# muzishen/RCDMs

Hardware: AMD Instinct MI355X
Metric: story-frames/sec (stage-2 UNet, 50-step DDIM, 512^2) (higher is better)
Workload: dtype f16; 1 GPU; PororoSV stage-2, 512x512, 50-step DDIM, CFG 2.0, batch=1 story x 5 frames per GPU, ctx 85x768, random-init 1276.9M-param UNet3D; stories_per_gpu=1, latent=64, ddim_steps=50, parallelism=story-replicas x1

## Files before the change

rcdms_amd/csrc/rowff.hip:

```cpp
#include "common.h"
#include "pp_sync.h"
#include <type_traits>

#ifndef RCDM_FF_ABLATE
#define RCDM_FF_ABLATE 0
#endif

namespace {

enum { TAIL_FF = 0, TAIL_N1 = 1, TAIL_FFP = 2, TAIL_N3 = 3 };

struct RowArgs {
  const f16* a_in;
  const f16* res;
  f16* tok;
  f16* out;
  const f16* wstream;
  const float* a_bias;
  const float* ln_g;
  const float* ln_b;
  const float* pe;
  const float* b1p;
  const float* b2;
  const f16* z_res;
  const float* z_bias;
  const float* gn_stat;
  const float* gn_g;
  const float* gn_b;
  int M, lda, ldr, ldt, ldo, ldz;
  int rows_per_frame, frames;
  int gn_G, gn_rows;
  float eps;
};

template <int C, int NW, int R, int PD, bool HAS_A, bool A_RES, bool LN_PE, int TAIL>
__global__ __launch_bounds__(NW * 64) void row_chain_kernel(const RowArgs p) {
  constexpr int NK = C / 32;
  constexpr int NOF = C / 16;
  constexpr int CHF = 2 * NK;
  constexpr int CHB = CHF * 1024;
  constexpr int NG = C / 8;
  constexpr int NCH_A = HAS_A ? NK : 0;
  constexpr bool IS_FF = TAIL == TAIL_FF || TAIL == TAIL_FFP;
  constexpr int NCH_T = IS_FF ? 3 * NG + (TAIL == TAIL_FFP ? NK : 0) : TAIL * NK;
  constexpr int NCH = NCH_A + NCH_T;
  constexpr int NT = NW * 64;
  constexpr int PPW = CHF / NW;
  static_assert(CHF % NW == 0, "chunk fragments must divide over the waves");
  static_assert(NOF == CHF && CHF % PD == 0 && CHF >= 20 && NOF % 2 == 0, "chunk geometry");
  constexpr int PAR0 = R * CHB;
  constexpr int RS = 2 * C + 16;
  static_assert(NW * 16 * RS <= R * CHB, "epilogue staging exceeds the ring");
  extern __shared__ __attribute__((aligned(16))) char smem[];

  const int t = threadIdx.x, lane = t & 63;
  const int wave = __builtin_amdgcn_readfirstlane(t >> 6);
  const int l15 = lane & 15, kg = lane >> 4;
  const int row0 = blockIdx.x * (NW * 16) + wave * 16;
  const int row = row0 + l15;
  const bool live = row < p.M;
  const int oG = HAS_A ? C : 0, oB = oG + C, oPE = oB + C, oT = oPE + (LN_PE ? p.frames * C : 0);
  const int oZ = oT + (IS_FF ? 8 * C : 0);
  const int oGN = oZ + (TAIL == TAIL_FFP ? 2 * C : 0);
  const int npar = oGN;

  const __amdgpu_buffer_rsrc_t rsrcW =
      __builtin_amdgcn_make_buffer_rsrc((void*)p.wstream, 0, (unsigned)NCH * CHB, 0x00020000);
  int dma_voff = lane * 16;
  auto issue_chunk = [&](int c, int slot) __attribute__((always_inline)) {
#pragma unroll
    for (int i = 0; i < PPW; ++i) {
      const int piece = wave * PPW + i;
      const unsigned voff = c < NCH ? (unsigned)dma_voff : 0x80000000u;
      __builtin_amdgcn_raw_ptr_buffer_load_lds(rsrcW, (__attribute__((address_space(3))) void*)(smem + slot * CHB + piece * 1024),
                                               16, voff, c < NCH ? c * CHB + piece * 1024 : 0, 0, 0);
// ... 24 lines not shown
  f32x4 bq[NB4_PER];
#pragma unroll
  for (int i = 0; i < NB4_PER; ++i) {
    const int idx = min(i * NT + t, npar / 4 - 1) * 4;
    const float* src;
    if (HAS_A && idx < oG) src = p.a_bias + idx;
    else if (idx < oB) src = p.ln_g + (idx - oG);
    else if (idx < oPE) src = p.ln_b + (idx - oB);
    else if (LN_PE && idx < oT) src = p.pe + (idx - oPE);
    else if (idx < oZ) src = p.b1p + (idx - oT);
    else if (idx < oZ + C) src = p.b2 + (idx - oZ);
    else src = p.z_bias + (idx - oZ - C);
    bq[i] = *(const f32x4*)src;
  }
  float gn_sc = 0.f, gn_sh = 0.f;
  constexpr bool CAN_GN = HAS_A && !A_RES;
  static_assert(NT == 2 * C, "one thread per (sample slot, channel)");
  if (CAN_GN && p.gn_stat) {
    const int j = t >= C ? 1 : 0, ch = t - j * C;
    const int nsamp = (p.M + p.gn_rows - 1) / p.gn_rows;
    const int smp = min((int)(blockIdx.x * (NW * 16)) / p.gn_rows + j, nsamp - 1);
    const float* st = p.gn_stat + ((size_t)smp * p.gn_G + ch / (C / p.gn_G)) * 2;
    const float ga = p.gn_g[ch], be = p.gn_b[ch], mean = st[0], rstd = st[1];
    gn_sc = rstd * ga;
    gn_sh = __builtin_fmaf(-(mean * rstd), ga, be);
  }
  int cslot = 0;
#pragma unroll
  for (int c = 0; c < R - 1; ++c) issue_chunk(c, c);
#pragma unroll
  for (int i = 0; i < NB4_PER; ++i) {
    const int idx = i * NT + t;
    if (idx < npar / 4) *(f32x4*)(smem + PAR0 + 16 * idx) = bq[i];
  }
  const float* par = (const float*)(smem + PAR0);
  if (CAN_GN && p.gn_stat) {
    float* gp = (float*)(smem + PAR0) + oGN + (t >= C ? 2 * C : 0) + (t >= C ? t - C : t);
    gp[0] = gn_sc;
    gp[C] = gn_sh;
  }
  wait_lgkm0();
  wait_vm<(R - 2) * PPW>();
  tick_barrier();

  if (CAN_GN && p.gn_stat) {
    const int j = row0 / p.gn_rows - (int)(blockIdx.x * (NW * 16)) / p.gn_rows;
    const float* gs = par + oGN + (j > 0 ? 2 * C : 0) + 8 * kg;
#pragma unroll
    for (int s = 0; s < NK; ++s) {
      const f32x4 c0 = *(const f32x4*)(gs + 32 * s), c1 = *(const f32x4*)(gs + 32 * s + 4);
      const f32x4 h0 = *(const f32x4*)(gs + C + 32 * s), h1 = *(const f32x4*)(gs + C + 32 * s + 4);
      f16x8 y;
#pragma unroll
      for (int e = 0; e < 4; ++e) {
        float f0 = __builtin_fmaf((float)xr[s][e], c0[e], h0[e]), f1 = __builtin_fmaf((float)xr[s][4 + e], c1[e], h1[e]);
        asm volatile("" : "+v"(f0), "+v"(f1));
        y[e] = (f16)f0;
        y[4 + e] = (f16)f1;
      }
      xr[s] = y;
    }
  }
// ... 70 lines not shown
      for (int j = 0; j < 8; ++j) s += (float)src[k][j];
    s += __shfl_xor(s, 16, 64);
    s += __shfl_xor(s, 32, 64);
    const float mean = s * (1.0f / C);
    float q = 0.f;
#pragma unroll
    for (int k = 0; k < NK; ++k)
#pragma unroll
      for (int j = 0; j < 8; ++j) {
        const float d = (float)src[k][j] - mean;
        q += d * d;
      }
    q += __shfl_xor(q, 16, 64);
    q += __shfl_xor(q, 32, 64);
    const float rstd = rsqrtf(q * (1.0f / C) + p.eps);
    const float* pep = LN_PE ? par + oPE + (((live ? row : 0) / p.rows_per_frame) % p.frames) * C : par;
#pragma unroll
    for (int k = 0; k < NK; ++k) {
      const int ch = 32 * k + 8 * kg;
      const f32x4 g0 = *(const f32x4*)(par + oG + ch), g1 = *(const f32x4*)(par + oG + ch + 4);
      f32x4 b0 = *(const f32x4*)(par + oB + ch), b1 = *(const f32x4*)(par + oB + ch + 4);
      if (LN_PE) {
        b0 += *(const f32x4*)(pep + ch);
        b1 += *(const f32x4*)(pep + ch + 4);
      }
      f16x8 y;
#pragma unroll
      for (int j = 0; j < 4; ++j) {
        y[j] = (f16)(((float)src[k][j] - mean) * rstd * g0[j] + b0[j]);
        y[4 + j] = (f16)(((float)src[k][4 + j] - mean) * rstd * g1[j] + b1[j]);
      }
// ... 46 lines not shown
        } else {
#pragma unroll
          for (int e = 0; e < 4; ++e) {
            pend[m][e] = (f16)acc[2 * m][e];
            pend[m][4 + e] = (f16)acc[2 * m + 1][e];
          }
        }
      }
      pend_col = grp * (C / 2);
    }
    wait_lgkm0();
    wait_vm<0>();
    store_pend();
  };

  if constexpr (!IS_FF) {
    gemm_groups(std::integral_constant<int, 2 * TAIL>{}, std::false_type{});
    return;
  } else {
    f32x4 oacc[NOF];
#pragma unroll
    for (int i = 0; i < NOF; ++i) oacc[i] = z4;
    struct GegluState { float bh, x, t, pl, ex; };
    auto geglu_slice = [&](int i, GegluState& st, const f32x4& ah, const f32x4& ag, int gp, f16* dst) __attribute__((always_inline)) {
      const int e = i / 5, stage = i - 5 * e;
      if (e >= 4) return;
      const float* bp = (const float*)(smem + PAR0 + (lane16 >> 8) * 16) + oT + gp * 32 + e;
      if (RCDM_FF_ABLATE & 32) {
        if (stage == 4) dst[e] = (f16)((ah[e] + bp[0]) * (ag[e] + bp[16]));
        return;
      }
// ... 120 lines not shown
          v.u = *(const uint4*)(st + r * RS + c8 * 16);
          const f32x4 a0 = *(const f32x4*)(p.b2 + c8 * 8), a1 = *(const f32x4*)(p.b2 + c8 * 8 + 4);
#pragma unroll
          for (int e = 0; e < 4; ++e) {
            o.e[e] = (f16)((float)v.e[e] + a0[e] + (float)rr[u].e[e]);
            o.e[4 + e] = (f16)((float)v.e[4 + e] + a1[e] + (float)rr[u].e[4 + e]);
          }
          *(uint4*)(p.out + (size_t)m * p.ldo + c8 * 8) = o.u;
        }
      }
    }
  }
}


__global__ void pack_pgemm_kernel(const float* __restrict__ w, int C, int n_blocks, f16* __restrict__ ws) {
  const int NK = C / 32, NOF = C / 16, HF = NOF / 2;
  const size_t per_block = (size_t)NOF * NK * 512, total = per_block * n_blocks;
  for (size_t idx = (size_t)blockIdx.x * blockDim.x + threadIdx.x; idx < total; idx += (size_t)gridDim.x * blockDim.x) {
    const int j = (int)(idx & 7), L = (int)((idx >> 3) & 63);
    const size_t fq = idx >> 9;
    const int blk = (int)(fq / (NOF * NK)), f = (int)(fq % (NOF * NK));
    const int h = f / (HF * NK), rem = f % (HF * NK), s = rem / HF, fi = rem % HF;
    const int i = h * HF + fi, r = L & 15, kq = L >> 4;
    const int n = blk * C + 32 * (i >> 1) + 8 * (r >> 2) + 4 * (i & 1) + (r & 3);
    ws[idx] = (f16)w[(size_t)n * C + 32 * s + 8 * kq + j];
  }
}

__global__ void pack_ff_stream_kernel(const float* __restrict__ w1, const float* __restrict__ b1, const float* __restrict__ w2,
                                      int C, f16* __restrict__ ws, float* __restrict__ b1p, int pperm) {
  const int NK = C / 32, CHF = 2 * NK;
  const size_t total = (size_t)12 * C * C;
  for (size_t idx = (size_t)blockIdx.x * blockDim.x + threadIdx.x; idx < total; idx += (size_t)gridDim.x * blockDim.x) {
    const int j = (int)(idx & 7), L = (int)((idx >> 3) & 63);
    const size_t fr = idx >> 9;
    const int f = (int)(fr % CHF), c = (int)(fr / CHF);
    int g, part;
// ... 17 lines not shown
      const int hid = 32 * g + (j < 4 ? 4 * kg + j : 16 + 4 * kg + (j - 4));
      const int n = pperm ? 32 * (f >> 1) + 8 * (l15 >> 2) + 4 * (f & 1) + (l15 & 3) : 16 * f + l15;
      v = w2[(size_t)n * (4 * C) + hid];
    }
    ws[idx] = (f16)v;
    if (idx < (size_t)8 * C) {
      const int q = (int)idx, gp = q >> 5, l = q & 31;
      const int hr = 16 * gp + (l & 15);
      b1p[q] = b1[l < 16 ? hr : 4 * C + hr];
    }
  }
}

template <bool HAS_A, bool A_RES, bool LN_PE, int TAIL>
int launch_chain(const RowArgs& a, hipStream_t stream) {
  constexpr int C = 320, NW = 10, R = 7, PD = 2;
  constexpr int CHB = 2 * (C / 32) * 1024;
  const int npar = (HAS_A ? C : 0) + 2 * C + (LN_PE ? a.frames * C : 0) + (TAIL == TAIL_FF || TAIL == TAIL_FFP ? 8 * C : 0) +
                   (TAIL == TAIL_FFP ? 2 * C : 0);
  const int lds = R * CHB + (npar + (a.gn_stat ? 4 * C : 0)) * 4;
  if (lds > 160 * 1024) return RCDM_ESHAPE;
  static bool attr_set[64] = {};
  if (rcdm_first_on_device(attr_set) &&
      hipFuncSetAttribute((const void*)row_chain_kernel<C, NW, R, PD, HAS_A, A_RES, LN_PE, TAIL>,
                          hipFuncAttributeMaxDynamicSharedMemorySize, 160 * 1024) != hipSuccess)
    return RCDM_ELAUNCH;
  const int nblocks = (a.M + NW * 16 - 1) / (NW * 16);
  hipLaunchKernelGGL((row_chain_kernel<C, NW, R, PD, HAS_A, A_RES, LN_PE, TAIL>), dim3(nblocks), dim3(NW * 64), lds, stream, a);
  return rcdm_check_launch();
}

inline unsigned grid_for(size_t n) {
  size_t g = (n + 255) / 256;
  return (unsigned)(g > 8192 ? 8192 : (g < 1 ? 1 : g));
}

inline bool misaligned16(const void* p) { return p && ((uintptr_t)p & 15); }
inline bool rows_overflow(int M, int ld) { return (size_t)M * (size_t)ld * 2 >= 0x7FFFFFFFull; }

}

extern "C" {

int rcdm_ff_fused_supported(int32_t C) { return C == 320 ? 1 : 0; }
int rcdm_rowchain_supported(int32_t C) { return C == 320 ? 1 : 0; }

int rcdm_rowchain_config_supported(int32_t C, int32_t tail, int32_t pe_frames) {
  if (C != 320 || tail < 0 || tail > 3) return 0;
  if (pe_frames < 0 || pe_frames > 8) return 0;
  if (pe_frames > 0 && (tail == 0 || tail == 2)) return 0;
  return 1;
}

size_t rcdm_ff_stream_bytes(int32_t C) { return C > 0 ? (size_t)24 * C * C : 0; }

size_t rcdm_rowchain_stream_bytes(int32_t C, int32_t tail) {
  if (C <= 0 || tail < 0 || tail > 3) return 0;
  return (size_t)2 * C * C * (1 + (tail == 0 ? 12 : tail == 2 ? 13 : tail));
}

int rcdm_pack_ff_stream(const float* w1, const float* b1, const float* w2, int32_t C, void* wstream, float* b1_packed,
                        void* stream) {
  if (!w1 || !b1 || !w2 || !wstream || !b1_packed || C <= 0) return RCDM_EINVAL;
  if (C % 32) return RCDM_ESHAPE;
  hipLaunchKernelGGL(pack_ff_stream_kernel, dim3(grid_for((size_t)12 * C * C)), dim3(256), 0, (hipStream_t)stream, w1, b1, w2, C,
                     (f16*)wstream, b1_packed, 0);
  return rcdm_check_launch();
}

int rcdm_pack_rowchain(const float* wa, int32_t C, int32_t tail, const float* wt, const float* w1, const float* b1,
                       const float* w2, void* wstream, float* b1_packed, void* stream) {
  if (!wa || !wstream || C <= 0) return RCDM_EINVAL;
  if (C % 32 || tail < 0 || tail > 3) return RCDM_ESHAPE;
  const bool ff = tail == 0 || tail == 2;
  if ((ff && (!w1 || !b1 || !w2 || !b1_packed)) || (tail != 0 && !wt)) return RCDM_EINVAL;
  f16* ws = (f16*)wstream;
  hipLaunchKernelGGL(pack_pgemm_kernel, dim3(grid_for((size_t)C * C)), dim3(256), 0, (hipStream_t)stream, wa, C, 1, ws);
  ws += (size_t)C * C;
  if (ff) {
    hipLaunchKernelGGL(pack_ff_stream_kernel, dim3(grid_for((size_t)12 * C * C)), dim3(256), 0, (hipStream_t)stream, w1, b1, w2, C,
                       ws, b1_packed, tail == 2 ? 1 : 0);
    ws += (size_t)12 * C * C;
  }
  if (tail != 0)
    hipLaunchKernelGGL(pack_pgemm_kernel, dim3(grid_for((size_t)(ff ? 1 : tail) * C * C)), dim3(256), 0, (hipStream_t)stream, wt, C,
                       ff ? 1 : tail, ws);
  return rcdm_check_launch();
}

int rcdm_ff_fused(const rcdm_ff_desc* d, const void* x, const float* ln_gamma, const float* ln_beta, const void* wstream,
                  const float* b1_packed, const float* b2, void* out, void* stream) {
  if (!d || !x || !ln_gamma || !ln_beta || !wstream || !b1_packed || !b2 || !out) return RCDM_EINVAL;
  if (d->M <= 0 || d->ldx < d->C || d->ldo < d->C || (d->ldx & 7) || (d->ldo & 7)) return RCDM_EINVAL;
  if (d->C != 320) return RCDM_ESHAPE;
  if (misaligned16(ln_gamma) || misaligned16(ln_beta) || misaligned16(b1_packed) || misaligned16(b2) || misaligned16(x) ||
      misaligned16(out) || misaligned16(wstream))
    return RCDM_EINVAL;
  if (rows_overflow(d->M, d->ldx) || rows_overflow(d->M, d->ldo)) return RCDM_ESHAPE;
  RowArgs a{};
  a.a_in = (const f16*)x; a.out = (f16*)out; a.wstream = (const f16*)wstream;
  a.ln_g = ln_gamma; a.ln_b = ln_beta; a.b1p = b1_packed; a.b2 = b2;
  a.M = d->M; a.lda = d->ldx; a.ldo = d->ldo; a.rows_per_frame = 1; a.frames = 1; a.eps = d->eps;
  return launch_chain<false, false, false, TAIL_FF>(a, (hipStream_t)stream);
}

int rcdm_rowchain(const rcdm_rowchain_desc* d, const void* a_in, const void* res, void* tok, const float* a_bias,
                  const float* ln_gamma, const float* ln_beta, const float* pe, const void* wstream, const float* b1_packed,
                  const float* b2, void* out, const float* gn_stat, const float* gn_gamma, const float* gn_beta,
                  const void* z_res, const float* z_bias, void* stream) {
  if (!d || !a_in || !tok || !a_bias || !ln_gamma || !ln_beta || !wstream || !out) return RCDM_EINVAL;
  const int ncol = d->tail == 0 || d->tail == 2 ? d->C : d->tail * d->C;
  if (d->M <= 0 || d->lda < d->C || d->ldt < d->C || d->ldo < ncol || ((d->lda | d->ldt | d->ldo) & 7)) return RCDM_EINVAL;
  if (res && (d->ldr < d->C || (d->ldr & 7))) return RCDM_EINVAL;
  if (pe && (d->rows_per_frame <= 0 || d->frames <= 0 || d->frames > 8)) return RCDM_EINVAL;
  if ((d->tail == 0 || d->tail == 2) && (!b1_packed || !b2)) return RCDM_EINVAL;
  if (d->C != 320 || d->tail < 0 || d->tail > 3) return RCDM_ESHAPE;
  if (!rcdm_rowchain_config_supported(d->C, d->tail, pe ? d->frames : 0)) return RCDM_ESHAPE;
  if (misaligned16(a_bias) || misaligned16(ln_gamma) || misaligned16(ln_beta) || misaligned16(pe) || misaligned16(b1_packed) ||
      misaligned16(b2) || misaligned16(z_bias) || misaligned16(gn_gamma) || misaligned16(gn_beta) || misaligned16(a_in) ||
      misaligned16(res) || misaligned16(tok) || misaligned16(out) || misaligned16(z_res) || misaligned16(wstream))
    return RCDM_EINVAL;
  if (rows_overflow(d->M, d->lda) || rows_overflow(d->M, d->ldt) || rows_overflow(d->M, d->ldo) ||
      (res && rows_overflow(d->M, d->ldr)) || (z_res && rows_overflow(d->M, d->ldz)))
    return RCDM_ESHAPE;
  if (d->tail == 2) {
    if (!res || pe || !z_res || !z_bias || d->ldz < d->C || (d->ldz & 7)) return RCDM_EINVAL;
  }
  if (gn_stat) {
    if (res || !gn_gamma || !gn_beta || d->gn_groups <= 0 || d->gn_rows <= 0) return RCDM_EINVAL;
    if (d->C % d->gn_groups || d->gn_rows % 16 || d->gn_rows < 160) return RCDM_ESHAPE;
  }
  RowArgs a{};
  a.a_in = (const f16*)a_in; a.res = (const f16*)res; a.tok = (f16*)tok; a.out = (f16*)out; a.wstream = (const f16*)wstream;
  a.a_bias = a_bias; a.ln_g = ln_gamma; a.ln_b = ln_beta; a.pe = pe; a.b1p = b1_packed; a.b2 = b2;
  a.M = d->M; a.lda = d->lda; a.ldr = d->ldr; a.ldt = d->ldt; a.ldo = d->ldo;
  a.rows_per_frame = pe ? d->rows_per_frame : 1; a.frames = pe ? d->frames : 1; a.eps = d->eps;
  a.z_res = (const f16*)z_res; a.z_bias = z_bias; a.ldz = d->ldz;
  a.gn_stat = gn_stat; a.gn_g = gn_gamma; a.gn_b = gn_beta; a.gn_G = d->gn_groups; a.gn_rows = d->gn_rows;
  hipStream_t s = (hipStream_t)stream;
#define RCDM_CHAIN(T)                                                                  \
  (res ? (pe ? launch_chain<true, true, true, T>(a, s) : launch_chain<true, true, false, T>(a, s)) \
       : (pe ? launch_chain<true, false, true, T>(a, s) : launch_chain<true, false, false, T>(a, s)))
  switch (d->tail) {
    case 0: return RCDM_CHAIN(TAIL_FF);
    case 1: return RCDM_CHAIN(TAIL_N1);
    case 2: return launch_chain<true, true, false, TAIL_FFP>(a, s);
    default: return RCDM_CHAIN(TAIL_N3);
  }
#undef RCDM_CHAIN
}

}
```

rcdms_amd/emit_blocks.py:

```python
import torch

from . import hip
from . import switches as SW
from .emit_ops import (XATTN_MAX_KEYS, assert_no_pending_gn, conv3x3_wino_ok, emit_conv3x3, emit_conv3x3_wino, emit_flash_attn, emit_gemm,
                       emit_groupnorm, emit_groupnorm_stats, emit_layernorm, emit_temporal_attn, emit_xattn, emit_xattn_pack, gemm_lnx_ok)
from .packer import MSUB_SCORE_LIMIT, attn_score_bound
from .plan import Rows, _NS


def emit_resnet(plan, w, x, geo, temb, out, eps=1e-5, groups=32, out_scale=1.0, dup_rows=0, out_gn=None):
    g = geo
    u1, u2 = getattr(w, "wino1", None) is not None, getattr(w, "wino2", None) is not None
    rv = (temb[0], temb[1], temb[2], g.f * g.hw)
    cross = (g.b, g.f * g.hw, groups)
    assert not (u1 or u2) or (not dup_rows and x.C == w.cin)
    h1 = plan.rows("res_h1", g.M, w.cout)
    res = x

    def unfolded_shortcut():
        if u2 or w.shortcut is None:
            return x
        sc = plan.rows("res_sc", g.M, w.cout)
        emit_gemm(plan, x, w.shortcut, w.cout, w.cin, sc, bias=w.sb)
        return sc
# ... 62 lines not shown

    def __le__(self, other):
        return self.value() <= other

    def __gt__(self, other):
        return self.value() > other

    def __int__(self):
        return self.value()

    def __repr__(self):
        return str(self.value())


CHAIN_MIN_ROWS = _ChainMinRows()


def emit_rowchain(plan, a_in, res, tok, a_bias, ln, pe, stream, tail, out, rows_per_frame=1, frames=1, b2=None, gn=None,
                  z=None):
    ws, b1p = stream
    M, C = a_in.M, a_in.C
    assert_no_pending_gn(plan, "a row-chain launch")
    d = hip.RowChainDesc(M, C, a_in.ld, res.ld if res is not None else 0, tok.ld, out.ld, tail, rows_per_frame, frames, 1e-5,
                         gn[3] if gn else 0, gn[4] if gn else 0, z[0].ld if z else 0)

    def op():
        hip.rowchain(d, a_in.ptr, res.ptr if res is not None else 0, tok.ptr, a_bias.data_ptr(), ln[0].data_ptr(),
                     ln[1].data_ptr(), pe.data_ptr() if pe is not None else 0, ws.data_ptr(),
                     b1p.data_ptr() if b1p is not None else 0, b2.data_ptr() if b2 is not None else 0, out.ptr,
                     gn_stat=gn[0].ptr if gn else 0, gn_g=gn[1].data_ptr() if gn else 0, gn_b=gn[2].data_ptr() if gn else 0,
# ... 220 lines not shown
    a = plan.rows("norm", g.M, C)
    chained = (w.chains is not None and not prior_state and g.M >= CHAIN_MIN_ROWS and
               hip.rowchain_config_supported(C, 3, g.f))
    gn = None
    if prior_state:
        emit_layernorm(plan, x, w.prior_g, w.prior_b, a)
    elif chained and g.hw % 16 == 0 and g.hw >= 160:
        gn = emit_groupnorm_stats(plan, x, g.n_img, g.hw, w.gn_g, w.gn_b, 1e-6, groups)
    else:
        emit_groupnorm(plan, x, g.n_img, g.hw, w.gn_g, w.gn_b, 1e-6, False, a, groups)
    z, tok = (None, plan.rows("tok", g.M, C)) if chained else ffz_rows(plan, w, g.M, C, x, out)
    if chained:
        qkv = plan.rows("qkv", g.M, 3 * C)
        ao = plan.rows("attn_out", g.M, C)
        a0, a1 = w.attn
        emit_rowchain(plan, x if gn else a, None, tok, w.proj_in_b, (a0.ln_g, a0.ln_b), a0.pe, w.chains[0], 3, qkv, g.hw, g.f, gn=gn)
        emit_temporal_attn(plan, qkv, g.b, g.f, g.hw, heads, d_head, ao)
        emit_rowchain(plan, ao, tok, tok, a0.o_b, (a1.ln_g, a1.ln_b), a1.pe, w.chains[1], 3, qkv, g.hw, g.f)
        emit_temporal_attn(plan, qkv, g.b, g.f, g.hw, heads, d_head, ao)
        if w.chain_ffz is not None:
            emit_rowchain(plan, ao, tok, tok, a1.o_b, w.ff_ln, None, w.chain_ffz, 2, out, b2=w.ff2_b, z=(x, w.proj_out_b))
            return
        emit_rowchain(plan, ao, tok, tok, a1.o_b, w.ff_ln, None, w.chains[2], 0, tok, b2=w.ff2_b)
        emit_gemm(plan, tok, w.proj_out, C, C, out, bias=w.proj_out_b, residual=x)
        return
    want_stat = SW.LNX and g.M < CHAIN_MIN_ROWS
    st = emit_gemm(plan, a, w.proj_in, C, C, tok, bias=w.proj_in_b, stat=want_stat)
    for at in w.attn:
        qkv = plan.rows("qkv", g.M, 3 * C)
        lx = at.lnx
        if st is not None and lx is not None and gemm_lnx_ok(g.M, 3 * C, C, tok.ld, qkv.ld) and (at.pe is None or g.f <= at.pe.shape[0]):
            if at.pe is not None:
                tab = lx.tab[:g.f].repeat(g.b, 1).contiguous()
                emit_gemm(plan, tok, lx.W, 3 * C, C, qkv, rowvec=(tab, 0, 3 * C, g.hw), lnx=(st, lx.S))
# ... 13 lines not shown
```

rcdms_amd/packer.py:

```python
import math

import torch

from . import hip
from . import switches as SW
from .plan import _NS


class Packer:
    def __init__(self, sd, device):
        self.sd, self.device = sd, torch.device(device)
        self._tmp = []

    def f32(self, key):
        t = self.sd[key].detach().to(self.device, torch.float32).contiguous()
        return t

    def has(self, key):
        return key in self.sd

    def vec(self, key):
        return self.f32(key)

    def mat_f16(self, *keys):
# ... 118 lines not shown
        wa = self.f32(wa_key).reshape(Cc, Cc).contiguous()
        ws = torch.empty(hip.rowchain_stream_bytes(Cc, tail), dtype=torch.uint8, device=self.device)
        if tail == 2:
            w1, b1, w2 = (self.f32(k) for k in ff_keys)
            wz = self.f32(wt_keys[0])
            if w1.shape != (8 * Cc, Cc) or w2.shape != (Cc, 4 * Cc) or wz.numel() != Cc * Cc:
                return None
            wz = wz.reshape(Cc, Cc).contiguous()
            b1p = torch.empty(8 * Cc, dtype=torch.float32, device=self.device)
            hip.pack_rowchain(wa.data_ptr(), Cc, 2, wz.data_ptr(), w1.data_ptr(), b1.data_ptr(), w2.data_ptr(), ws.data_ptr(),
                              b1p.data_ptr())
            self._tmp += [wa, wz, w1, b1, w2]
            return ws, b1p
        if tail:
            wt = torch.cat([self.f32(k) for k in wt_keys], dim=0).contiguous()
            if tuple(wt.shape) != (tail * Cc, Cc):
                return None
            hip.pack_rowchain(wa.data_ptr(), Cc, tail, wt.data_ptr(), 0, 0, 0, ws.data_ptr(), 0)
            self._tmp += [wa, wt]
            return ws, None
        w1, b1, w2 = (self.f32(k) for k in ff_keys)
        if w1.shape != (8 * Cc, Cc) or w2.shape != (Cc, 4 * Cc):
            return None
        b1p = torch.empty(8 * Cc, dtype=torch.float32, device=self.device)
        hip.pack_rowchain(wa.data_ptr(), Cc, 0, 0, w1.data_ptr(), b1.data_ptr(), w2.data_ptr(), ws.data_ptr(), b1p.data_ptr())
        self._tmp += [wa, w1, b1, w2]
        return ws, b1p

    def done(self):
        torch.cuda.synchronize(self.device)
        self._tmp.clear()
# ... 130 lines not shown
    for i in range(n_attn):
        a = b + f"attention_blocks.{i}."
        pe = pk.f32(a + "pos_encoder.pe")[0].contiguous() if pk.has(a + "pos_encoder.pe") else None
        ln_g, ln_b = pk.vec(b + f"norms.{i}.weight"), pk.vec(b + f"norms.{i}.bias")
        w.attn.append(_NS(
            ln_g=ln_g, ln_b=ln_b, pe=pe,
            qkv=pk.mat_f16(a + "to_q.weight", a + "to_k.weight", a + "to_v.weight"),
            lnx=pk.lnx_mat((a + "to_q.weight", a + "to_k.weight", a + "to_v.weight"), ln_g, ln_b, pe=pe) if lnx else None,
            o=pk.mat_f16(a + "to_out.0.weight"), o_b=pk.vec(a + "to_out.0.bias")))
    w.ff_ln = (pk.vec(b + "ff_norm.weight"), pk.vec(b + "ff_norm.bias"))
    w.lnx_ff = pk.lnx_geglu(b + "ff.net.0.proj.weight", b + "ff.net.0.proj.bias", *w.ff_ln) if lnx else None
    w.ff1, w.ff1_b = pk.geglu(b + "ff.net.0.proj.weight", b + "ff.net.0.proj.bias")
    w.ff2, w.ff2_b = pk.mat_f16(b + "ff.net.2.weight"), pk.vec(b + "ff.net.2.bias")
    w.ff_stream = pk.ff_stream(b + "ff.net.0.proj.weight", b + "ff.net.0.proj.bias", b + "ff.net.2.weight")
    w.ffz = pk.ffz(b + "ff.net.2.weight", b + "ff.net.2.bias", p + "proj_out.weight", p + "proj_out.bias") if lnx else None
    w.chains = w.chain_ffz = None
    if n_attn == 2:
        a0, a1 = b + "attention_blocks.0.", b + "attention_blocks.1."
        qkv = lambda a: (a + "to_q.weight", a + "to_k.weight", a + "to_v.weight")
        ch = [pk.chain(p + "proj_in.weight", 3, wt_keys=qkv(a0)), pk.chain(a0 + "to_out.0.weight", 3, wt_keys=qkv(a1)),
              pk.chain(a1 + "to_out.0.weight", 0,
                       ff_keys=(b + "ff.net.0.proj.weight", b + "ff.net.0.proj.bias", b + "ff.net.2.weight"))]
        if all(c is not None for c in ch) and all(at.pe is not None for at in w.attn):
            w.chains = ch
            w.chain_ffz = pk.chain(a1 + "to_out.0.weight", 2, wt_keys=(p + "proj_out.weight",),
                                   ff_keys=(b + "ff.net.0.proj.weight", b + "ff.net.0.proj.bias", b + "ff.net.2.weight"))
    return w
```

rcdms_amd/switches.py:

```python
import os


def _on(name, default="1"):
    return os.environ.get(name, default) != "0"


SC_FOLD = _on("RCDM_SC_FOLD")
UP2 = _on("RCDM_UP2")
GN_PRESTAT = _on("RCDM_GN_PRESTAT")
LNX = _on("RCDM_LNX")
FFZ = _on("RCDM_FFZ")
FF_FUSE = _on("RCDM_FF_FUSE")
ROW_CHAIN = _on("RCDM_ROWCHAIN")
RANK1_CTX = _on("RCDM_RANK1_CTX")
_w = os.environ.get("RCDM_WINO", "le32").strip()
WINO_MAX_SIDE = int(_w[2:]) if _w.startswith("le") else 0
WINO_MIN_SIDE = 8
WINO_MIN_C = int(os.environ.get("RCDM_WINO_MIN_C", "640"))
WINO = tuple(int(v) for v in _w.split(",") if v.strip().isdigit() and int(v) > 0) if not _w.startswith("le") else ()


def wino_side(H, W):
    if H % 2 or W % 2:
        return False
    return (min(H, W) >= WINO_MIN_SIDE and max(H, W) <= WINO_MAX_SIDE) if WINO_MAX_SIDE else (H == W and H in WINO)


UP9 = _on("RCDM_UP9")
OUT_TAPS = _on("RCDM_OUT_TAPS")
_vf = os.environ.get("RCDM_VAE_FLASH", "auto").strip().lower()
VAE_FLASH = _vf if _vf in ("0", "1") else "auto"
CHAIN_MIN_ROWS = os.environ.get("RCDM_CHAIN_MIN_ROWS")

TABLE = {
    "RCDM_SC_FOLD": SC_FOLD, "RCDM_UP2": UP2, "RCDM_GN_PRESTAT": GN_PRESTAT, "RCDM_LNX": LNX, "RCDM_FFZ": FFZ,
    "RCDM_FF_FUSE": FF_FUSE, "RCDM_ROWCHAIN": ROW_CHAIN, "RCDM_RANK1_CTX": RANK1_CTX, "RCDM_WINO": _w, "RCDM_WINO_MIN_C": WINO_MIN_C, "RCDM_UP9": UP9, "RCDM_OUT_TAPS": OUT_TAPS, "RCDM_CHAIN_MIN_ROWS": CHAIN_MIN_ROWS,
    "RCDM_VAE_FLASH": VAE_FLASH,
}
```

Baseline: 6.189 story-frames/s.

## Fuse temporal motion attention into the row-chain QKV kernel via frame-major tiling

Adds a frame-major TAIL_ATT variant of the row-chain kernel for C=320. Each block holds all 5 frames of a spatial row group across its waves, computes the Q/K/V projection, exchanges K/V through LDS, and runs the 8-head, 5-frame softmax attention in-kernel. This removes the QKV round trip through global memory and the separate temporal-attention launches for the first two motion attention blocks. The cost is a smaller weight ring (5 slots instead of 7), an extra LDS exchange region, a reordered weight packing, and tighter shape restrictions (5 frames, rows per frame a multiple of 16).

Measured after the change: 6.275 story-frames/s (median of 6 runs). 1.01x the previous value.

```diff
diff --git a/rcdms_amd/csrc/rowff.hip b/rcdms_amd/csrc/rowff.hip
--- a/rcdms_amd/csrc/rowff.hip
+++ b/rcdms_amd/csrc/rowff.hip
@@ -8,7 +8,7 @@
 
 namespace {
 
-enum { TAIL_FF = 0, TAIL_N1 = 1, TAIL_FFP = 2, TAIL_N3 = 3 };
+enum { TAIL_FF = 0, TAIL_N1 = 1, TAIL_FFP = 2, TAIL_N3 = 3, TAIL_ATT = 4 };
 
 struct RowArgs {
   const f16* a_in;
@@ -31,6 +31,7 @@
   int rows_per_frame, frames;
   int gn_G, gn_rows;
   float eps;
+  float att_scale;
 };
 
 template <int C, int NW, int R, int PD, bool HAS_A, bool A_RES, bool LN_PE, int TAIL>
@@ -42,7 +43,8 @@
   constexpr int NG = C / 8;
   constexpr int NCH_A = HAS_A ? NK : 0;
   constexpr bool IS_FF = TAIL == TAIL_FF || TAIL == TAIL_FFP;
-  constexpr int NCH_T = IS_FF ? 3 * NG + (TAIL == TAIL_FFP ? NK : 0) : TAIL * NK;
+  constexpr bool FM = TAIL == TAIL_ATT;
+  constexpr int NCH_T = IS_FF ? 3 * NG + (TAIL == TAIL_FFP ? NK : 0) : (FM ? 3 : TAIL) * NK;
   constexpr int NCH = NCH_A + NCH_T;
   constexpr int NT = NW * 64;
   constexpr int PPW = CHF / NW;
@@ -50,15 +52,28 @@
   static_assert(NOF == CHF && CHF % PD == 0 && CHF >= 20 && NOF % 2 == 0, "chunk geometry");
   constexpr int PAR0 = R * CHB;
   constexpr int RS = 2 * C + 16;
-  static_assert(NW * 16 * RS <= R * CHB, "epilogue staging exceeds the ring");
+  static_assert(!IS_FF || NW * 16 * RS <= R * CHB, "epilogue staging exceeds the ring");
+  constexpr int XOFF = PAR0 + 3 * C * 4, XW = (NK / 2) * 1024;
+  static_assert(!FM || (HAS_A && NW == 10 && (5 * C + NW * 2 * C) * 4 <= NW * XW), "frame-major chain geometry");
   extern __shared__ __attribute__((aligned(16))) char smem[];
 
   const int t = threadIdx.x, lane = t & 63;
   const int wave = __builtin_amdgcn_readfirstlane(t >> 6);
   const int l15 = lane & 15, kg = lane >> 4;
-  const int row0 = blockIdx.x * (NW * 16) + wave * 16;
+  int row0_ = blockIdx.x * (NW * 16) + wave * 16, fm_gps = 1, fm_ngrp = 0;
+  bool fm_live = true;
+  const int fm_f = wave % 5;
+  if constexpr (FM) {
+    fm_gps = p.rows_per_frame >> 4;
+    fm_ngrp = (p.M / (5 * p.rows_per_frame)) * fm_gps;
+    const int grp = 2 * blockIdx.x + wave / 5;
+    fm_live = grp < fm_ngrp;
+    const int g2 = fm_live ? grp : 0, b = g2 / fm_gps;
+    row0_ = (b * 5 + fm_f) * p.rows_per_frame + 16 * (g2 - b * fm_gps);
+  }
+  const int row0 = row0_;
   const int row = row0 + l15;
-  const bool live = row < p.M;
+  const bool live = FM ? fm_live : row < p.M;
   const int oG = HAS_A ? C : 0, oB = oG + C, oPE = oB + C, oT = oPE + (LN_PE ? p.frames * C : 0);
   const int oZ = oT + (IS_FF ? 8 * C : 0);
   const int oGN = oZ + (TAIL == TAIL_FFP ? 2 * C : 0);
@@ -113,9 +128,24 @@
     bq[i] = *(const f32x4*)src;
   }
   float gn_sc = 0.f, gn_sh = 0.f;
+  float fm_sc[FM ? 5 : 1], fm_sh[FM ? 5 : 1];
   constexpr bool CAN_GN = HAS_A && !A_RES;
   static_assert(NT == 2 * C, "one thread per (sample slot, channel)");
-  if (CAN_GN && p.gn_stat) {
+  if constexpr (FM && CAN_GN) {
+    if (p.gn_stat) {
+      const int j0 = t >= C ? 1 : 0, ch = t - j0 * C;
+      const float ga = p.gn_g[ch], be = p.gn_b[ch];
+#pragma unroll
+      for (int i = 0; i < 5; ++i) {
+        const int j = 2 * i + j0;
+        const int smp = (min(2 * (int)blockIdx.x + j / 5, fm_ngrp - 1) / fm_gps) * 5 + j % 5;
+        const float* st = p.gn_stat + ((size_t)smp * p.gn_G + ch / (C / p.gn_G)) * 2;
+        const float mean = st[0], rstd = st[1];
+        fm_sc[i] = rstd * ga;
+        fm_sh[i] = __builtin_fmaf(-(mean * rstd), ga, be);
+      }
+    }
+  } else if (CAN_GN && p.gn_stat) {
     const int j = t >= C ? 1 : 0, ch = t - j * C;
     const int nsamp = (p.M + p.gn_rows - 1) / p.gn_rows;
     const int smp = min((int)(blockIdx.x * (NW * 16)) / p.gn_rows + j, nsamp - 1);
@@ -133,7 +163,16 @@
     if (idx < npar / 4) *(f32x4*)(smem + PAR0 + 16 * idx) = bq[i];
   }
   const float* par = (const float*)(smem + PAR0);
-  if (CAN_GN && p.gn_stat) {
+  if constexpr (FM && CAN_GN) {
+    if (p.gn_stat) {
+#pragma unroll
+      for (int i = 0; i < 5; ++i) {
+        float* gp = (float*)(smem + PAR0) + oGN + (2 * i + (t >= C ? 1 : 0)) * 2 * C + (t >= C ? t - C : t);
+        gp[0] = fm_sc[i];
+        gp[C] = fm_sh[i];
+      }
+    }
+  } else if (CAN_GN && p.gn_stat) {
     float* gp = (float*)(smem + PAR0) + oGN + (t >= C ? 2 * C : 0) + (t >= C ? t - C : t);
     gp[0] = gn_sc;
     gp[C] = gn_sh;
@@ -143,8 +182,8 @@
   tick_barrier();
 
   if (CAN_GN && p.gn_stat) {
-    const int j = row0 / p.gn_rows - (int)(blockIdx.x * (NW * 16)) / p.gn_rows;
-    const float* gs = par + oGN + (j > 0 ? 2 * C : 0) + 8 * kg;
+    const int j = FM ? wave : row0 / p.gn_rows - (int)(blockIdx.x * (NW * 16)) / p.gn_rows;
+    const float* gs = par + oGN + (FM ? j * 2 * C : j > 0 ? 2 * C : 0) + 8 * kg;
 #pragma unroll
     for (int s = 0; s < NK; ++s) {
       const f32x4 c0 = *(const f32x4*)(gs + 32 * s), c1 = *(const f32x4*)(gs + 32 * s + 4);
@@ -245,7 +284,7 @@
     q += __shfl_xor(q, 16, 64);
     q += __shfl_xor(q, 32, 64);
     const float rstd = rsqrtf(q * (1.0f / C) + p.eps);
-    const float* pep = LN_PE ? par + oPE + (((live ? row : 0) / p.rows_per_frame) % p.frames) * C : par;
+    const float* pep = !LN_PE ? par : FM ? par + oPE + fm_f * C : par + oPE + (((live ? row : 0) / p.rows_per_frame) % p.frames) * C;
 #pragma unroll
     for (int k = 0; k < NK; ++k) {
       const int ch = 32 * k + 8 * kg;
@@ -322,7 +361,136 @@
     store_pend();
   };
 
-  if constexpr (!IS_FF) {
+  if constexpr (FM) {
+    constexpr int HG = NK / 2;
+    char* const X = smem + XOFF;
+    const int kgq = lane16 >> 8, xme = wave * XW + lane16, xgrp = (wave / 5) * 5 * XW + lane16;
+    const bool c1 = kgq == 0, c2 = kgq <= 1, c3 = kgq <= 2;
+    f16x8 qh[HG], pend[HG], oh[HG];
+    f32x4 acc[NOF / 2];
+    float sc[4][5], o8[8];
+    auto round_to = [&](f16x8 (&dst)[HG]) __attribute__((always_inline)) {
+#pragma unroll
+      for (int m = 0; m < HG; ++m)
+#pragma unroll
+        for (int e = 0; e < 4; ++e) {
+          dst[m][e] = (f16)acc[2 * m][e];
+          dst[m][4 + e] = (f16)acc[2 * m + 1][e];
+        }
+    };
+    auto xput = [&]() __attribute__((always_inline)) {
+#pragma unroll
+      for (int m = 0; m < HG; ++m) *(f16x8*)(X + xme + m * 1024) = pend[m];
+    };
+    auto xget = [&](int fp, int m) __attribute__((always_inline)) -> f16x8 { return *(const f16x8*)(X + xgrp + fp * XW + m * 1024); };
+    auto score_item = [&](int fp, int m) __attribute__((always_inline)) {
+      const f16x8 kv = xget(fp, m);
+      float d = 0.f;
+#pragma unroll
+      for (int e = 0; e < 8; e += 2)
+        d = __builtin_amdgcn_fdot2(f16x2{qh[m][e], qh[m][e + 1]}, f16x2{kv[e], kv[e + 1]}, d, false);
+      if (m == 0) {
+        sc[0][fp] = d; sc[1][fp] = 0.f; sc[2][fp] = 0.f; sc[3][fp] = 0.f;
+        asm volatile("" : "+v"(sc[0][fp]));
+      } else if (m == 4) {
+        sc[3][fp] += d;
+        asm volatile("" : "+v"(sc[3][fp]));
+      } else {
+        const float lo = (m == 1 ? c1 : m == 2 ? c2 : c3) ? d : 0.f;
+        sc[m - 1][fp] += lo;
+        sc[m][fp] += d - lo;
+        asm volatile("" : "+v"(sc[m - 1][fp]), "+v"(sc[m][fp]));
+      }
+    };
+    auto reduce_item = [&](int h, int fp) __attribute__((always_inline)) {
+      float v = sc[h][fp];
+      v += __shfl_xor(v, 16, 64);
+      v += __shfl_xor(v, 32, 64);
+      asm volatile("" : "+v"(v));
+      sc[h][fp] = v;
+    };
+    auto softmax_head = [&](int h) __attribute__((always_inline)) {
+      float mx = sc[h][0] * p.att_scale;
+#pragma unroll
+      for (int j = 0; j < 5; ++j) {
+        sc[h][j] *= p.att_scale;
+        mx = fmaxf(mx, sc[h][j]);
+      }
+      float sum = 0.f;
+#pragma unroll
+      for (int j = 0; j < 5; ++j) {
+        sc[h][j] = __expf(sc[h][j] - mx);
+        sum += sc[h][j];
+      }
+      const float inv = __builtin_amdgcn_rcpf(sum);
+#pragma unroll
+      for (int j = 0; j < 5; ++j) sc[h][j] *= inv;
+      asm volatile("" : "+v"(sc[h][0]), "+v"(sc[h][1]), "+v"(sc[h][2]), "+v"(sc[h][3]), "+v"(sc[h][4]));
+    };
+    auto pv_item = [&](int m, int fp) __attribute__((always_inline)) {
+      const f16x8 vv = xget(fp, m);
+      const float pj = m == 0 ? sc[0][fp] : m == 4 ? sc[3][fp] : (m == 1 ? c1 : m == 2 ? c2 : c3) ? sc[m - 1][fp] : sc[m][fp];
+#pragma unroll
+      for (int e = 0; e < 8; ++e) o8[e] = __builtin_fmaf(pj, (float)vv[e], fp == 0 ? 0.f : o8[e]);
+      if (fp == 4) {
+#pragma unroll
+        for (int e = 0; e < 8; ++e) oh[m][e] = (f16)o8[e];
+        asm volatile("" : "+v"(oh[m]));
+      } else {
+        asm volatile("" : "+v"(o8[0]), "+v"(o8[1]), "+v"(o8[2]), "+v"(o8[3]), "+v"(o8[4]), "+v"(o8[5]), "+v"(o8[6]), "+v"(o8[7]));
+      }
+    };
+    auto store_o = [&](int half) __attribute__((always_inline)) {
+      if (live) {
+        f16* op = p.out + (size_t)row * p.ldo + half * (C / 2) + 8 * kgq;
+#pragma unroll
+        for (int m = 0; m < HG; ++m) st16(op + 32 * m, oh[m]);
+      }
+    };
+    auto group = [&](auto hh_c, auto grp_c) __attribute__((always_inline)) {
+      constexpr int hh = decltype(hh_c)::value, grp = decltype(grp_c)::value;
+#pragma unroll
+      for (int cc = 0; cc < HG; ++cc)
+        run_chunk(
+            [&](int i, f16x8 w) __attribute__((always_inline)) {
+              const int s = 2 * cc + i / (NOF / 2), fi = i % (NOF / 2);
+              acc[fi] = mm(w, xr[s], s == 0 ? z4 : acc[fi]);
+            },
+            [&](int i) __attribute__((always_inline)) {
+              if constexpr (grp == 2) {
+                if (cc >= 1 && cc <= 3 && i < (cc == 3 ? 5 : 10)) score_item(2 * (cc - 1) + i / 5, i % 5);
+                if (cc == 4) reduce_item(i / 5, i % 5);
+              } else if constexpr (grp == 0 && hh == 1) {
+                if (cc == 0 && i % 5 == 2) softmax_head(i / 5);
+                if (cc >= 1 && cc <= 3 && i < (cc == 3 ? 5 : 10)) pv_item(2 * (cc - 1) + i / 5, i % 5);
+              }
+            },
+            [&]() __attribute__((always_inline)) {
+              if (cc == 0 && (grp == 2 || (grp == 0 && hh == 1))) xput();
+              if (cc == 0 && grp == 1 && hh == 1) store_o(0);
+            });
+      if constexpr (grp == 0) round_to(qh); else round_to(pend);
+    };
+    using I0 = std::integral_constant<int, 0>;
+    using I1 = std::integral_constant<int, 1>;
+    using I2 = std::integral_constant<int, 2>;
+    group(I0{}, I0{}); group(I0{}, I1{}); group(I0{}, I2{});
+    group(I1{}, I0{}); group(I1{}, I1{}); group(I1{}, I2{});
+#pragma unroll
+    for (int h = 0; h < 4; ++h) softmax_head(h);
+    wait_lgkm0();
+    wait_vm<0>();
+    tick_barrier();
+    xput();
+    wait_lgkm0();
+    tick_barrier();
+#pragma unroll
+    for (int m = 0; m < HG; ++m)
+#pragma unroll
+      for (int fp = 0; fp < 5; ++fp) pv_item(m, fp);
+    store_o(1);
+    return;
+  } else if constexpr (!IS_FF) {
     gemm_groups(std::integral_constant<int, 2 * TAIL>{}, std::false_type{});
     return;
   } else {
@@ -473,14 +641,21 @@
 }
 
 
-__global__ void pack_pgemm_kernel(const float* __restrict__ w, int C, int n_blocks, f16* __restrict__ ws) {
+__global__ void pack_pgemm_kernel(const float* __restrict__ w, int C, int n_blocks, f16* __restrict__ ws, int by_half) {
   const int NK = C / 32, NOF = C / 16, HF = NOF / 2;
   const size_t per_block = (size_t)NOF * NK * 512, total = per_block * n_blocks;
   for (size_t idx = (size_t)blockIdx.x * blockDim.x + threadIdx.x; idx < total; idx += (size_t)gridDim.x * blockDim.x) {
     const int j = (int)(idx & 7), L = (int)((idx >> 3) & 63);
     const size_t fq = idx >> 9;
-    const int blk = (int)(fq / (NOF * NK)), f = (int)(fq % (NOF * NK));
-    const int h = f / (HF * NK), rem = f % (HF * NK), s = rem / HF, fi = rem % HF;
+    int blk = (int)(fq / (NOF * NK));
+    const int f = (int)(fq % (NOF * NK));
+    int h = f / (HF * NK);
+    const int rem = f % (HF * NK), s = rem / HF, fi = rem % HF;
+    if (by_half) {
+      const int gs = 2 * blk + h;
+      blk = gs % 3;
+      h = gs / 3;
+    }
     const int i = h * HF + fi, r = L & 15, kq = L >> 4;
     const int n = blk * C + 32 * (i >> 1) + 8 * (r >> 2) + 4 * (i & 1) + (r & 3);
     ws[idx] = (f16)w[(size_t)n * C + 32 * s + 8 * kq + j];
@@ -528,11 +703,12 @@
 
 template <bool HAS_A, bool A_RES, bool LN_PE, int TAIL>
 int launch_chain(const RowArgs& a, hipStream_t stream) {
-  constexpr int C = 320, NW = 10, R = 7, PD = 2;
+  constexpr int C = 320, NW = 10, PD = 2;
+  constexpr int R = TAIL == TAIL_ATT ? 5 : 7;
   constexpr int CHB = 2 * (C / 32) * 1024;
   const int npar = (HAS_A ? C : 0) + 2 * C + (LN_PE ? a.frames * C : 0) + (TAIL == TAIL_FF || TAIL == TAIL_FFP ? 8 * C : 0) +
                    (TAIL == TAIL_FFP ? 2 * C : 0);
-  const int lds = R * CHB + (npar + (a.gn_stat ? 4 * C : 0)) * 4;
+  const int lds = TAIL == TAIL_ATT ? R * CHB + 3 * C * 4 + NW * (C / 64) * 1024 : R * CHB + (npar + (a.gn_stat ? 4 * C : 0)) * 4;
   if (lds > 160 * 1024) return RCDM_ESHAPE;
   static bool attr_set[64] = {};
   if (rcdm_first_on_device(attr_set) &&
@@ -560,8 +736,9 @@
 int rcdm_rowchain_supported(int32_t C) { return C == 320 ? 1 : 0; }
 
 int rcdm_rowchain_config_supported(int32_t C, int32_t tail, int32_t pe_frames) {
-  if (C != 320 || tail < 0 || tail > 3) return 0;
+  if (C != 320 || tail < 0 || tail > 4) return 0;
   if (pe_frames < 0 || pe_frames > 8) return 0;
+  if (tail == 4 && pe_frames != 0 && pe_frames != 5) return 0;
   if (pe_frames > 0 && (tail == 0 || tail == 2)) return 0;
   return 1;
 }
@@ -569,8 +746,8 @@
 size_t rcdm_ff_stream_bytes(int32_t C) { return C > 0 ? (size_t)24 * C * C : 0; }
 
 size_t rcdm_rowchain_stream_bytes(int32_t C, int32_t tail) {
-  if (C <= 0 || tail < 0 || tail > 3) return 0;
-  return (size_t)2 * C * C * (1 + (tail == 0 ? 12 : tail == 2 ? 13 : tail));
+  if (C <= 0 || tail < 0 || tail > 4) return 0;
+  return (size_t)2 * C * C * (1 + (tail == 0 ? 12 : tail == 2 ? 13 : tail == 4 ? 3 : tail));
 }
 
 int rcdm_pack_ff_stream(const float* w1, const float* b1, const float* w2, int32_t C, void* wstream, float* b1_packed,
@@ -585,20 +762,21 @@
 int rcdm_pack_rowchain(const float* wa, int32_t C, int32_t tail, const float* wt, const float* w1, const float* b1,
                        const float* w2, void* wstream, float* b1_packed, void* stream) {
   if (!wa || !wstream || C <= 0) return RCDM_EINVAL;
-  if (C % 32 || tail < 0 || tail > 3) return RCDM_ESHAPE;
+  if (C % 32 || tail < 0 || tail > 4) return RCDM_ESHAPE;
   const bool ff = tail == 0 || tail == 2;
   if ((ff && (!w1 || !b1 || !w2 || !b1_packed)) || (tail != 0 && !wt)) return RCDM_EINVAL;
   f16* ws = (f16*)wstream;
-  hipLaunchKernelGGL(pack_pgemm_kernel, dim3(grid_for((size_t)C * C)), dim3(256), 0, (hipStream_t)stream, wa, C, 1, ws);
+  hipLaunchKernelGGL(pack_pgemm_kernel, dim3(grid_for((size_t)C * C)), dim3(256), 0, (hipStream_t)stream, wa, C, 1, ws, 0);
   ws += (size_t)C * C;
   if (ff) {
     hipLaunchKernelGGL(pack_ff_stream_kernel, dim3(grid_for((size_t)12 * C * C)), dim3(256), 0, (hipStream_t)stream, w1, b1, w2, C,
                        ws, b1_packed, tail == 2 ? 1 : 0);
     ws += (size_t)12 * C * C;
   }
+  const int nt = ff ? 1 : tail == 4 ? 3 : tail;
   if (tail != 0)
-    hipLaunchKernelGGL(pack_pgemm_kernel, dim3(grid_for((size_t)(ff ? 1 : tail) * C * C)), dim3(256), 0, (hipStream_t)stream, wt, C,
-                       ff ? 1 : tail, ws);
+    hipLaunchKernelGGL(pack_pgemm_kernel, dim3(grid_for((size_t)nt * C * C)), dim3(256), 0, (hipStream_t)stream, wt, C, nt, ws,
+                       tail == 4 ? 1 : 0);
   return rcdm_check_launch();
 }
 
@@ -623,12 +801,16 @@
                   const float* b2, void* out, const float* gn_stat, const float* gn_gamma, const float* gn_beta,
                   const void* z_res, const float* z_bias, void* stream) {
   if (!d || !a_in || !tok || !a_bias || !ln_gamma || !ln_beta || !wstream || !out) return RCDM_EINVAL;
-  const int ncol = d->tail == 0 || d->tail == 2 ? d->C : d->tail * d->C;
+  const int ncol = d->tail == 0 || d->tail == 2 || d->tail == 4 ? d->C : d->tail * d->C;
   if (d->M <= 0 || d->lda < d->C || d->ldt < d->C || d->ldo < ncol || ((d->lda | d->ldt | d->ldo) & 7)) return RCDM_EINVAL;
   if (res && (d->ldr < d->C || (d->ldr & 7))) return RCDM_EINVAL;
   if (pe && (d->rows_per_frame <= 0 || d->frames <= 0 || d->frames > 8)) return RCDM_EINVAL;
   if ((d->tail == 0 || d->tail == 2) && (!b1_packed || !b2)) return RCDM_EINVAL;
-  if (d->C != 320 || d->tail < 0 || d->tail > 3) return RCDM_ESHAPE;
+  if (d->C != 320 || d->tail < 0 || d->tail > 4) return RCDM_ESHAPE;
+  if (d->tail == 4) {
+    if (d->rows_per_frame <= 0 || d->frames <= 0) return RCDM_EINVAL;
+    if (d->frames != 5 || d->rows_per_frame % 16 || d->M % (5 * d->rows_per_frame)) return RCDM_ESHAPE;
+  }
   if (!rcdm_rowchain_config_supported(d->C, d->tail, pe ? d->frames : 0)) return RCDM_ESHAPE;
   if (misaligned16(a_bias) || misaligned16(ln_gamma) || misaligned16(ln_beta) || misaligned16(pe) || misaligned16(b1_packed) ||
       misaligned16(b2) || misaligned16(z_bias) || misaligned16(gn_gamma) || misaligned16(gn_beta) || misaligned16(a_in) ||
@@ -642,13 +824,15 @@
   }
   if (gn_stat) {
     if (res || !gn_gamma || !gn_beta || d->gn_groups <= 0 || d->gn_rows <= 0) return RCDM_EINVAL;
-    if (d->C % d->gn_groups || d->gn_rows % 16 || d->gn_rows < 160) return RCDM_ESHAPE;
+    if (d->C % d->gn_groups || d->gn_rows % 16) return RCDM_ESHAPE;
+    if (d->tail == 4 ? d->gn_rows != d->rows_per_frame : d->gn_rows < 160) return RCDM_ESHAPE;
   }
   RowArgs a{};
   a.a_in = (const f16*)a_in; a.res = (const f16*)res; a.tok = (f16*)tok; a.out = (f16*)out; a.wstream = (const f16*)wstream;
   a.a_bias = a_bias; a.ln_g = ln_gamma; a.ln_b = ln_beta; a.pe = pe; a.b1p = b1_packed; a.b2 = b2;
   a.M = d->M; a.lda = d->lda; a.ldr = d->ldr; a.ldt = d->ldt; a.ldo = d->ldo;
-  a.rows_per_frame = pe ? d->rows_per_frame : 1; a.frames = pe ? d->frames : 1; a.eps = d->eps;
+  a.rows_per_frame = pe || d->tail == 4 ? d->rows_per_frame : 1; a.frames = pe || d->tail == 4 ? d->frames : 1; a.eps = d->eps;
+  a.att_scale = (float)(1.0 / sqrt((double)(d->C / 8)));
   a.z_res = (const f16*)z_res; a.z_bias = z_bias; a.ldz = d->ldz;
   a.gn_stat = gn_stat; a.gn_g = gn_gamma; a.gn_b = gn_beta; a.gn_G = d->gn_groups; a.gn_rows = d->gn_rows;
   hipStream_t s = (hipStream_t)stream;
@@ -659,7 +843,8 @@
     case 0: return RCDM_CHAIN(TAIL_FF);
     case 1: return RCDM_CHAIN(TAIL_N1);
     case 2: return launch_chain<true, true, false, TAIL_FFP>(a, s);
-    default: return RCDM_CHAIN(TAIL_N3);
+    case 3: return RCDM_CHAIN(TAIL_N3);
+    default: return RCDM_CHAIN(TAIL_ATT);
   }
 #undef RCDM_CHAIN
 }
diff --git a/rcdms_amd/emit_blocks.py b/rcdms_amd/emit_blocks.py
--- a/rcdms_amd/emit_blocks.py
+++ b/rcdms_amd/emit_blocks.py
@@ -100,6 +100,7 @@
 
 
 CHAIN_MIN_ROWS = _ChainMinRows()
+MOTION_FUSE_MIN_ROWS = _ChainMinRows()
 
 
 def emit_rowchain(plan, a_in, res, tok, a_bias, ln, pe, stream, tail, out, rows_per_frame=1, frames=1, b2=None, gn=None,
@@ -350,10 +351,15 @@
         qkv = plan.rows("qkv", g.M, 3 * C)
         ao = plan.rows("attn_out", g.M, C)
         a0, a1 = w.attn
-        emit_rowchain(plan, x if gn else a, None, tok, w.proj_in_b, (a0.ln_g, a0.ln_b), a0.pe, w.chains[0], 3, qkv, g.hw, g.f, gn=gn)
-        emit_temporal_attn(plan, qkv, g.b, g.f, g.hw, heads, d_head, ao)
-        emit_rowchain(plan, ao, tok, tok, a0.o_b, (a1.ln_g, a1.ln_b), a1.pe, w.chains[1], 3, qkv, g.hw, g.f)
-        emit_temporal_attn(plan, qkv, g.b, g.f, g.hw, heads, d_head, ao)
+        if (w.chains_att is not None and g.f == 5 and heads == 8 and g.hw % 16 == 0 and g.M >= MOTION_FUSE_MIN_ROWS and
+                hip.rowchain_config_supported(C, 4, g.f)):
+            emit_rowchain(plan, x if gn else a, None, tok, w.proj_in_b, (a0.ln_g, a0.ln_b), a0.pe, w.chains_att[0], 4, ao, g.hw, g.f, gn=gn)
+            emit_rowchain(plan, ao, tok, tok, a0.o_b, (a1.ln_g, a1.ln_b), a1.pe, w.chains_att[1], 4, ao, g.hw, g.f)
+        else:
+            emit_rowchain(plan, x if gn else a, None, tok, w.proj_in_b, (a0.ln_g, a0.ln_b), a0.pe, w.chains[0], 3, qkv, g.hw, g.f, gn=gn)
+            emit_temporal_attn(plan, qkv, g.b, g.f, g.hw, heads, d_head, ao)
+            emit_rowchain(plan, ao, tok, tok, a0.o_b, (a1.ln_g, a1.ln_b), a1.pe, w.chains[1], 3, qkv, g.hw, g.f)
+            emit_temporal_attn(plan, qkv, g.b, g.f, g.hw, heads, d_head, ao)
         if w.chain_ffz is not None:
             emit_rowchain(plan, ao, tok, tok, a1.o_b, w.ff_ln, None, w.chain_ffz, 2, out, b2=w.ff2_b, z=(x, w.proj_out_b))
             return
diff --git a/rcdms_amd/packer.py b/rcdms_amd/packer.py
--- a/rcdms_amd/packer.py
+++ b/rcdms_amd/packer.py
@@ -156,7 +156,7 @@
             return ws, b1p
         if tail:
             wt = torch.cat([self.f32(k) for k in wt_keys], dim=0).contiguous()
-            if tuple(wt.shape) != (tail * Cc, Cc):
+            if tuple(wt.shape) != ((3 if tail == 4 else tail) * Cc, Cc):
                 return None
             hip.pack_rowchain(wa.data_ptr(), Cc, tail, wt.data_ptr(), 0, 0, 0, ws.data_ptr(), 0)
             self._tmp += [wa, wt]
@@ -317,7 +317,7 @@
     w.ff2, w.ff2_b = pk.mat_f16(b + "ff.net.2.weight"), pk.vec(b + "ff.net.2.bias")
     w.ff_stream = pk.ff_stream(b + "ff.net.0.proj.weight", b + "ff.net.0.proj.bias", b + "ff.net.2.weight")
     w.ffz = pk.ffz(b + "ff.net.2.weight", b + "ff.net.2.bias", p + "proj_out.weight", p + "proj_out.bias") if lnx else None
-    w.chains = w.chain_ffz = None
+    w.chains = w.chain_ffz = w.chains_att = None
     if n_attn == 2:
         a0, a1 = b + "attention_blocks.0.", b + "attention_blocks.1."
         qkv = lambda a: (a + "to_q.weight", a + "to_k.weight", a + "to_v.weight")
@@ -326,6 +326,8 @@
                        ff_keys=(b + "ff.net.0.proj.weight", b + "ff.net.0.proj.bias", b + "ff.net.2.weight"))]
         if all(c is not None for c in ch) and all(at.pe is not None for at in w.attn):
             w.chains = ch
+            if SW.MOTION_FUSE and hip.rowchain_config_supported(C, 4, 5):
+                w.chains_att = [pk.chain(p + "proj_in.weight", 4, wt_keys=qkv(a0)), pk.chain(a0 + "to_out.0.weight", 4, wt_keys=qkv(a1))]
             w.chain_ffz = pk.chain(a1 + "to_out.0.weight", 2, wt_keys=(p + "proj_out.weight",),
                                    ff_keys=(b + "ff.net.0.proj.weight", b + "ff.net.0.proj.bias", b + "ff.net.2.weight"))
     return w
diff --git a/rcdms_amd/switches.py b/rcdms_amd/switches.py
--- a/rcdms_amd/switches.py
+++ b/rcdms_amd/switches.py
@@ -12,6 +12,7 @@
 FFZ = _on("RCDM_FFZ")
 FF_FUSE = _on("RCDM_FF_FUSE")
 ROW_CHAIN = _on("RCDM_ROWCHAIN")
+MOTION_FUSE = _on("RCDM_MOTION_FUSE")
 RANK1_CTX = _on("RCDM_RANK1_CTX")
 _w = os.environ.get("RCDM_WINO", "le32").strip()
 WINO_MAX_SIDE = int(_w[2:]) if _w.startswith("le") else 0
@@ -34,6 +35,6 @@
 
 TABLE = {
     "RCDM_SC_FOLD": SC_FOLD, "RCDM_UP2": UP2, "RCDM_GN_PRESTAT": GN_PRESTAT, "RCDM_LNX": LNX, "RCDM_FFZ": FFZ,
-    "RCDM_FF_FUSE": FF_FUSE, "RCDM_ROWCHAIN": ROW_CHAIN, "RCDM_RANK1_CTX": RANK1_CTX, "RCDM_WINO": _w, "RCDM_WINO_MIN_C": WINO_MIN_C, "RCDM_UP9": UP9, "RCDM_OUT_TAPS": OUT_TAPS, "RCDM_CHAIN_MIN_ROWS": CHAIN_MIN_ROWS,
+    "RCDM_FF_FUSE": FF_FUSE, "RCDM_ROWCHAIN": ROW_CHAIN, "RCDM_MOTION_FUSE": MOTION_FUSE, "RCDM_RANK1_CTX": RANK1_CTX, "RCDM_WINO": _w, "RCDM_WINO_MIN_C": WINO_MIN_C, "RCDM_UP9": UP9, "RCDM_OUT_TAPS": OUT_TAPS, "RCDM_CHAIN_MIN_ROWS": CHAIN_MIN_ROWS,
     "RCDM_VAE_FLASH": VAE_FLASH,
 }
```
